# dwofk/fast-depth

Measured on NVIDIA H100. Metric: depth-maps/sec @224x224 b64, higher is better.
Workload: dtype f16

## Files before the change

### fastdepth_b200/_lib.py

```python
import ctypes
import os

HERE = os.path.dirname(os.path.abspath(__file__))
LIB_PATH = os.environ.get('FD_B200_LIB') or os.path.join(HERE, 'libfastdepth_b200.so')

FD_F32, FD_F16, FD_BF16 = 0, 1, 2
FD_STAGE_STEM, FD_STAGE_DWPW, FD_STAGE_HEAD, FD_STAGE_CONV, FD_STAGE_DECONV, FD_STAGE_UPCONV = 0, 1, 2, 3, 4, 5
FD_ACT_RELU, FD_ACT_RELU6 = 0, 1


class StageDesc(ctypes.Structure):
    _fields_ = [(n, ctypes.c_int32) for n in
                ('kind', 'c_in', 'c_out', 'ksize', 'stride', 'act', 'upsample', 'skip_src', 'skip_mode')]


_c_int_p = ctypes.POINTER(ctypes.c_int)
_c_float_p = ctypes.POINTER(ctypes.c_float)
_c_double_p = ctypes.POINTER(ctypes.c_double)
_vp = ctypes.c_void_p

SIGNATURES = {
    'fd_abi_version': (ctypes.c_int, []),
    'fd_last_error': (ctypes.c_char_p, []),
    'fd_plan_create': (ctypes.c_int, [ctypes.POINTER(StageDesc), ctypes.c_int, ctypes.c_int, ctypes.c_int,
# ... 9 lines not shown
    'fd_stage_buffer': (ctypes.c_int, [_vp, ctypes.c_int, ctypes.c_int, ctypes.POINTER(_vp),
                                       _c_int_p, _c_int_p, _c_int_p, _c_int_p, _c_int_p]),
    'fd_plan_launches_per_forward': (ctypes.c_int, [_vp, _c_int_p]),
    'fd_plan_workspace_bytes': (ctypes.c_int, [_vp, ctypes.POINTER(ctypes.c_size_t)]),
    'fd_plan_step_count': (ctypes.c_int, [_vp, _c_int_p]),
    'fd_plan_step_info': (ctypes.c_int, [_vp, ctypes.c_int, _c_int_p, _c_double_p, _c_double_p,
                                         ctypes.c_char_p, ctypes.c_int]),
    'fd_plan_step_macs': (ctypes.c_int, [_vp, ctypes.c_int, _c_double_p, _c_double_p]),
    'fd_plan_time_steps': (ctypes.c_int, [_vp, _vp, _vp, _vp, ctypes.c_int, ctypes.c_int, ctypes.c_int, _c_float_p]),
    'fd_plan_trace_stage': (ctypes.c_int, [_vp, ctypes.c_int, _vp, _vp, ctypes.POINTER(ctypes.c_uint64), ctypes.c_int,
                                           _c_int_p, _c_int_p]),
    'fd_debug_block_plan': (ctypes.c_int, [ctypes.c_int] * 8 + [_c_int_p, ctypes.c_int]),
    'fd_debug_conv_plan': (ctypes.c_int, [ctypes.c_int] * 7 + [_c_int_p, ctypes.c_int]),
    'fd_debug_convt_plan': (ctypes.c_int, [ctypes.c_int] * 8 + [_c_int_p, ctypes.c_int]),
    'fd_debug_pw_tf32x3_plan': (ctypes.c_int, [ctypes.c_int] * 7 + [_c_int_p, ctypes.c_int]),
    'fd_debug_conv_tf32x3_plan': (ctypes.c_int, [ctypes.c_int] * 9 + [_c_int_p, ctypes.c_int]),
    'fd_metrics_accumulate': (ctypes.c_int, [_vp, _vp, ctypes.c_int, ctypes.c_int, ctypes.c_int, _vp,
                                             ctypes.c_int, _vp]),
    'fd_nyu_val_gather': (ctypes.c_int, [_vp, _vp, _vp, _vp] + [ctypes.c_int] * 6 + [_vp, _vp, ctypes.c_int, _vp]),
    'fd_plan_destroy': (None, [_vp]),
}

_lib = None


def load():
    global _lib
    if _lib is not None:
        return _lib
    if not os.path.exists(LIB_PATH):
# ... 19 lines not shown
```

### fastdepth_b200/csrc/fd_api.cu

```cuda
#include <algorithm>
#include <cstring>
#include <functional>
#include <string>
#include <vector>

#include "fd_block_plan.h"
#include "fd_conv_plan.h"
#include "fd_common.cuh"

namespace fd {

BlockPlanOut block_tc_debug_plan(int ksize, int stride, int h_out, int w_out, int n, int c_in, int c_out, int head);
ConvPlanOut conv_tc_debug_plan(int kind, int ksize, int h_out, int w_out, int n, int c_in, int c_out, int n_sms);
ConvPlanOut pw_tf32x3_debug_plan(int h_out, int w_out, int n, int c_in, int c_out, int upsample, int n_sms);
ConvPlanOut conv_tc_tf32x3_debug_plan(int kind, int ksize, int h_out, int w_out, int n, int c_in, int c_out, int upsample,
                                      int n_sms);

static thread_local std::string g_last_error;
void set_error(const std::string& msg) { g_last_error = msg; }
int fail(int code, const std::string& msg) {
    g_last_error = msg;
    return code;
}

int launch_stem(int dtype, const void* x, void* out, const float* w, const float* scale, const float* bias,
                const StageGeom& g, cudaStream_t st);
int launch_dw(int dtype, const BlockArgs& a, cudaStream_t st);
int launch_pw(int dtype, const BlockArgs& a, cudaStream_t st);
int launch_conv(int dtype, const void* in, const void* w, void* out, const float* scale, const float* bias, const StageGeom& g,
// ... 29 lines not shown
const char* stem_tc_name(StemTcPlan* sp);
struct ConvTcPlan;
bool conv_tc_supported(int dtype, const StageGeom& g, int kind);
int conv_tc_prepare(int dtype, int kind, const StageGeom& g, const void* in, const void* w, const float* scale_dev,
                    const float* bias_dev, void* out, const TcLaunchOpts& opts, ConvTcPlan** res);
int conv_tc_launch(ConvTcPlan* cp, cudaStream_t st);
void conv_tc_destroy(ConvTcPlan* cp);
const char* conv_tc_name(ConvTcPlan* cp);
bool pw_tf32x3_supported(const StageGeom& g);
bool conv_tc_tf32x3_supported(const StageGeom& g, int kind);
int conv_tc_tf32x3_prepare(int kind, const StageGeom& g, const void* in, const float* w_split, const float* scale_dev,
                           const float* bias_dev, void* out, const TcLaunchOpts& opts, ConvTcPlan** res);
int pw_tf32x3_prepare(const StageGeom& g, const void* mid, const float* w_split, const float* scale_dev, const float* bias_dev,
                      void* out, int out_pitch, int reduce, const TcLaunchOpts& opts, ConvTcPlan** res);
int tf32_split_weights(const float* w, size_t count, float* dst);
size_t block_tc_param_bytes(BlockTcPlan* bp);
size_t chain_tc_param_bytes(ChainTcPlan* cp);
size_t stem_tc_param_bytes(StemTcPlan* sp);
size_t conv_tc_param_bytes(ConvTcPlan* cp);

static size_t dtype_size(int dtype) { return dtype == FD_F32 ? 4 : 2; }
static bool is_phased(int kind) { return kind == FD_STAGE_DECONV || kind == FD_STAGE_UPCONV; }
static bool is_conv(int kind) { return kind == FD_STAGE_CONV || is_phased(kind); }

struct Stage {
    fd_stage_desc d{};
    StageGeom g{};
    int out_h = 0, out_w = 0;
    void* out = nullptr;
    void* out_alloc = nullptr;
// ... 39 lines not shown
};

}

using namespace fd;

struct fd_plan {
    int n = 0, h = 0, w = 0, dtype = 0, device = 0, n_sms = 132;
    std::vector<Stage> stages;
    std::vector<StepSet*> sets;
    unsigned long long set_clock = 0;
    int opt_path = 1, opt_fold_head = 1, opt_graph = 1, opt_tma_epilogue = 1, opt_inplace_skip = 1, opt_pdl = 0, opt_wait_sleep_ns = 0;
    int opt_chain = 1;
    int opt_cluster = 1;
    int opt_tf32x3 = 0;
    size_t workspace_bytes = 0;
    size_t split_bytes = 0;
    struct PipeSlot { void* x = nullptr; void* y = nullptr; cudaEvent_t up = nullptr, done = nullptr, down = nullptr; bool busy = false; };
    PipeSlot pipe[3];
    cudaStream_t pipe_h2d = nullptr, pipe_run = nullptr, pipe_d2h = nullptr;
    unsigned long long pipe_next = 0;
    void* stage_x = nullptr;
    void* stage_y = nullptr;
    cudaEvent_t last_done = nullptr;
    cudaStream_t last_stream = nullptr;
    bool last_stream_set = false;
    void* l2_flush = nullptr;
    size_t l2_flush_bytes = 0;
    struct GraphEntry { const void* x; void* y; int n; cudaGraphExec_t exec; unsigned long long stamp; };
    std::vector<GraphEntry> graphs;
    unsigned long long graph_clock = 0;
    int graph_misses = 0;
};
static const size_t kMaxGraphs = 8;
static const size_t kMaxStepSets = 8;

namespace fd {

struct DeviceGuard {
    int prev = -1;
    bool ok = true;
    explicit DeviceGuard(int dev) {
        if (cudaGetDevice(&prev) != cudaSuccess) { ok = false; return; }
        if (prev != dev && cudaSetDevice(dev) != cudaSuccess) ok = false;
    }
    ~DeviceGuard() {
        if (prev >= 0) cudaSetDevice(prev);
    }
};
// ... 218 lines not shown
            a.in = in;
            a.mid = s.mid;
            a.out = s.out;
            a.skip = (s.d.skip_src >= 0 && !s.d.skip_mode) ? R[s.d.skip_src].out_eff : nullptr;
            a.dw_w = s.dw_w; a.dw_scale = s.dw_scale; a.dw_bias = s.dw_bias;
            a.pw_w = s.pw_w; a.pw_scale = s.pw_scale; a.pw_bias = s.pw_bias;
            const double px_in = (double)sg.n * sg.h_in * sg.w_in, px_out = (double)sg.n * sg.h_out * sg.w_out;
            const double up = a.g.upsample ? 4.0 : 1.0;
            const double dw_macs = px_out * sg.c_in * sg.ksize * sg.ksize, pw_macs = px_out * sg.c_in * sg.c_out;
            const double w_bytes = (double)sg.c_in * sg.ksize * sg.ksize * 4 + 2.0 * sg.c_in * 4 +
                                   (double)sg.c_in * sg.c_out * es + 2.0 * sg.c_out * 4;
            const double fused_bytes = (px_in * sg.c_in + px_out * up * sg.c_out * (a.skip ? 2.0 : 1.0)) * es + w_bytes;
            const int dtype = p->dtype;
            const bool fuse_head = folded_here && p->opt_path == 1 && block_tc_supported(dtype, a.g, true);
            bool use_tc = p->opt_path == 1 && block_tc_supported(dtype, a.g, false);
            if (use_tc) {
                const bool tma_epi = p->opt_tma_epilogue != 0;
                if (tma_epi && p->opt_inplace_skip && a.skip != nullptr) { a.out = const_cast<void*>(a.skip); r.out_eff = a.out; }
                int rc = fuse_head ? block_tc_prepare(dtype, a, head.pw_w_f32, head.head_scale, head.head_bias, head.g.act, nullptr, false, lopts, &r.tc)
                                   : block_tc_prepare(dtype, a, nullptr, 0.f, 0.f, 0, nullptr, tma_epi && (a.skip == nullptr || a.skip == a.out), lopts, &r.tc);
                if (rc != FD_OK) return rc;
                ss->bytes += block_tc_param_bytes(r.tc);
                Step st;
                st.stage = i;
                st.name = block_tc_name(r.tc);
                st.macs = dw_macs + pw_macs + (fuse_head ? px_out * sg.c_out : 0.0);
                st.dw_macs = dw_macs;
                st.alg_bytes = fuse_head ? (px_in * sg.c_in + px_out * 4.0) * es + w_bytes + sg.c_out * 4.0 : fused_bytes;
                BlockTcPlan* tc = r.tc;
                st.run = [tc](cudaStream_t stream, const void*, void* y) { return block_tc_launch(tc, stream, y); };
// ... 260 lines not shown
    return FD_OK;
}

static int* option_slot(fd_plan* p, const char* name) {
    if (!p || !name) return nullptr;
    if (!strcmp(name, "path")) return &p->opt_path;
    if (!strcmp(name, "fold_head")) return &p->opt_fold_head;
    if (!strcmp(name, "graph")) return &p->opt_graph;
    if (!strcmp(name, "tma_epilogue")) return &p->opt_tma_epilogue;
    if (!strcmp(name, "inplace_skip")) return &p->opt_inplace_skip;
    if (!strcmp(name, "pdl")) return &p->opt_pdl;
    if (!strcmp(name, "wait_sleep_ns")) return &p->opt_wait_sleep_ns;
    if (!strcmp(name, "chain")) return &p->opt_chain;
    if (!strcmp(name, "cluster")) return &p->opt_cluster;
    if (!strcmp(name, "tf32x3")) return &p->opt_tf32x3;
    return nullptr;
}

int fd_plan_set_option(fd_plan* p, const char* name, int value) {
    int* slot = option_slot(p, name);
    if (!slot) return fail(FD_ERR_INVALID, std::string("unknown option: ") + (name ? name : "(null)"));
    const bool is_time = !strcmp(name, "wait_sleep_ns");
    if (is_time ? (value < 0 || value > 100000) : (value != 0 && value != 1))
        return fail(FD_ERR_INVALID, is_time ? "wait_sleep_ns must be in [0, 100000]" : "option value must be 0 or 1");
    if (*slot != value) { *slot = value; invalidate(p); }
    return FD_OK;
}

int fd_plan_get_option(fd_plan* p, const char* name, int* value) {
    int* slot = option_slot(p, name);
    if (!slot || !value) return fail(FD_ERR_INVALID, "unknown option or NULL value");
    *value = *slot;
    return FD_OK;
}

static int ensure_steps(fd_plan* p, int n, StepSet** out) {
    StepSet* ss = find_set(p, n);
    if (!ss) {
        if (p->sets.size() >= kMaxStepSets) {
// ... 296 lines not shown
    const int v[16] = {q.ok, q.splits, q.n_cta, q.items, q.kblocks, q.s_in, q.s_a, q.s_b, q.bn, q.nb, q.b_resident, q.n_stg,
                       q.smem_bytes, q.in_stage_stride, q.cs, q.dw_teams};
    for (int i = 0; i < 16; ++i) out[i] = v[i];
    return FD_OK;
}

int fd_debug_conv_plan(int ksize, int h_out, int w_out, int n, int c_in, int c_out, int n_sms, int* out, int cap) {
    if (!out || cap < 16) return fail(FD_ERR_INVALID, "need an int[16] output");
    const ConvPlanOut q = conv_tc_debug_plan(FD_STAGE_CONV, ksize, h_out, w_out, n, c_in, c_out, n_sms);
    const int v[16] = {q.ok, q.ni, q.th, q.tw, q.bn, q.stages, q.m_tiles, q.n_splits, q.items, q.waves, q.kblocks, q.smem_bytes,
                       q.useful_permille, (int)(q.cost > 2e9 ? 2e9 : q.cost), 0, 0};
    for (int i = 0; i < 16; ++i) out[i] = v[i];
    return FD_OK;
}

int fd_debug_pw_tf32x3_plan(int h_out, int w_out, int n, int c_in, int c_out, int upsample, int n_sms, int* out, int cap) {
    if (!out || cap < 16) return fail(FD_ERR_INVALID, "need an int[16] output");
    const ConvPlanOut q = pw_tf32x3_debug_plan(h_out, w_out, n, c_in, c_out, upsample, n_sms);
    const int v[16] = {q.ok, q.ni, q.th, q.tw, q.bn, q.stages, q.m_tiles, q.n_splits, q.items, q.waves, q.kblocks, q.smem_bytes,
                       q.useful_permille, (int)(q.cost > 2e9 ? 2e9 : q.cost), q.ok ? conv_stage_bytes_tf32x3(q.bn) : 0, 0};
    for (int i = 0; i < 16; ++i) out[i] = v[i];
    return FD_OK;
}

int fd_debug_conv_tf32x3_plan(int kind, int ksize, int h, int w, int n, int c_in, int c_out, int upsample, int n_sms, int* out,
                              int cap) {
    if (!out || cap < 44) return fail(FD_ERR_INVALID, "need an int[44] output");
    if (kind != FD_STAGE_CONV && !is_phased(kind)) return fail(FD_ERR_INVALID, "kind must be FD_STAGE_CONV, FD_STAGE_DECONV or FD_STAGE_UPCONV");
    const ConvPlanOut q = conv_tc_tf32x3_debug_plan(kind, ksize, h, w, n, c_in, c_out, upsample, n_sms);
    const int v[16] = {q.ok, q.ni, q.th, q.tw, q.bn, q.stages, q.m_tiles, q.n_splits, q.items, q.waves, q.kblocks, q.smem_bytes,
// ... 70 lines not shown
```

### fastdepth_b200/csrc/fd_block_tc.cu

```cuda
#include <cuda.h>

#include <cstdio>
#include <cstdlib>
#include <cstring>
#include <new>
#include <string>

#include "fd_block_plan.h"
#include "fd_tc_common.cuh"

namespace fd {

constexpr int TC_DW_WARPS = 8;
constexpr int TC_EPI_WARPS = 8;
constexpr int TC_WARP_EPI0 = 0, TC_WARP_DW0 = TC_EPI_WARPS;
constexpr int TC_WARP_TMA = TC_DW_WARPS + TC_EPI_WARPS;
constexpr int TC_THREADS = (TC_WARP_TMA + 1) * 32;
constexpr int TC_WARP_BCAST = TC_WARP_TMA + 1;
constexpr int TC_THREADS_CL = (TC_WARP_BCAST + 1) * 32;
constexpr int TC_NCH = 2;
constexpr int TC_KBLK = 64;
constexpr int TC_A_STAGE_BYTES = 128 * 128;
constexpr int TC_MAX_IN = 6, TC_MAX_A = 6, TC_MAX_B = 16;
static_assert(TC_MAX_A >= kPlanMaxACluster && TC_MAX_A >= kPlanMaxA && TC_MAX_IN >= kPlanMaxIn && TC_MAX_B >= kPlanMaxB, "barrier arrays cover the planner's ring depths");
// ... 769 lines not shown
    if (i < n_dst) dst[i] = i < n_src ? src[i] : 0.f;
}

static int padded_copy(const float* src, int n_src, int n_dst, float** out) {
    FD_CUDA_OK(cudaMalloc(out, (size_t)n_dst * 4));
    pad_copy_kernel<<<(n_dst + 255) / 256, 256>>>(src, *out, n_src, n_dst);
    FD_CUDA_OK(cudaGetLastError());
    return FD_OK;
}

static int block_wmc_auto(const StageGeom& g, const BlockPlanOut& po, int n_tiles) {
    (void)g; (void)po; (void)n_tiles;
    return 1;
}

int block_tc_prepare(int dtype, const BlockArgs& a, const float* head_w, float head_scale, float head_bias, int head_act,
                     void* head_out, bool tma_epilogue, const TcLaunchOpts& opts, BlockTcPlan** out) {
    PFN_encodeTiled encode = get_encode();
    if (!encode) return fail(FD_ERR_CUDA, "cuTensorMapEncodeTiled is not available from this driver");
    const StageGeom& g = a.g;
    BlockTcPlan* bp = new (std::nothrow) BlockTcPlan();
    if (!bp) return fail(FD_ERR_CUDA, "out of host memory");
    bp->dtype = dtype; bp->ks = g.ksize; bp->stride = g.stride; bp->tile = pick_tile(g);
    bp->opts = opts;
    {
        const char* e = getenv("FD_TC_NO_HALFK");
        bp->halfk = (g.c_in <= 32 && g.ksize == 3 && g.stride == 1 && bp->tile == 0 && !(e && *e == '1')) ? 1 : 0;
    }
    const int NI = bp->tile ? 2 : 1, TH = 8, TW = bp->tile ? 8 : 16;
    const int IH = (TH - 1) * g.stride + g.ksize, IW = (TW - 1) * g.stride + g.ksize;
    TcParams& p = bp->p;
    memset(&p, 0, sizeof(p));
    p.n = g.n; p.h_in = g.h_in; p.w_in = g.w_in; p.h_out = g.h_out; p.w_out = g.w_out; p.c_in = g.c_in; p.c_out = g.c_out;
    p.tiles_x = (g.w_out + TW - 1) / TW; p.tiles_y = (g.h_out + TH - 1) / TH;
    const int tiles_img = (g.n + NI - 1) / NI;
    const int n_tiles = p.tiles_x * p.tiles_y * tiles_img;
    p.kblocks = (g.c_in + TC_KBLK - 1) / TC_KBLK; p.cin_pad = p.kblocks * TC_KBLK;
    p.act = g.act; p.upsample = g.upsample;
    p.head = head_w != nullptr; p.head_act = head_act; p.head_scale = head_scale; p.head_bias = head_bias;
    p.skip = a.skip; p.out = a.out; p.head_out = head_out;
    p.out_pitch = g.out_pitch > 0 ? g.out_pitch : g.c_out; p.skip_pitch = g.skip_pitch > 0 ? g.skip_pitch : g.c_out;
    const int in_pitch = g.in_pitch > 0 ? g.in_pitch : g.c_in;

    BlockPlanIn pin{};
    pin.ksize = g.ksize; pin.stride = g.stride; pin.tile = bp->tile; pin.c_in = g.c_in; pin.c_out = g.c_out; pin.n_tiles = n_tiles;
    pin.head = p.head; pin.barrier_bytes = (int)sizeof(TcBarriers); pin.n_sms = opts.n_sms;
    pin.cluster = (opts.cluster && !bp->halfk) ? 0 : 1;
    { const char* e = getenv("FD_TC_DW_TEAMS"); pin.even_rings = (e && *e == '1') ? 0 : ((e && *e == '2') ? 1 : 2); }
    if (pin.even_rings == 2 && g.ksize == 5 && (g.c_in + TC_KBLK - 1) / TC_KBLK <= 2) pin.even_rings = 1;
    plan_env_knobs(pin);
    if (bp->halfk) pin.cluster = 1;
    const BlockPlanOut po = plan_block(pin);
    if (!po.ok) { delete bp; return fail(FD_ERR_UNSUPPORTED, "fused block does not fit shared memory"); }
    const int splits = po.splits;
    p.n_cta = po.n_cta; p.splits = po.splits; p.items = po.items;
    p.in_stage_bytes = po.in_stage_bytes; p.dwp_bytes = po.dwp_bytes; p.in_stage_stride = po.in_stage_stride; p.cpad_all = po.cpad_all;
    p.s_a = po.s_a; p.n_stg = po.n_stg; p.s_in = po.s_in; p.s_b = po.s_b; p.bn = po.bn; p.nb = po.nb;
    p.b_resident = po.b_resident; p.b_stage_bytes = po.b_stage_bytes;
    p.cs = po.cs; bp->tiles = n_tiles;
    { const char* e = getenv("FD_TC_EPI_HIGH"); p.epi_high = (e && *e) ? atoi(e) : 0; }
    p.dw_teams = po.dw_teams;
    p.wmc = 1;
    {
        const char* e = getenv("FD_TC_WMC");
        int want = e && *e ? atoi(e) : 0;
        if (!opts.cluster || bp->halfk) want = 1;
        if (want == 0) want = block_wmc_auto(g, po, n_tiles);
// ... 96 lines not shown
```

### fastdepth_b200/csrc/fd_conv_plan.h

```cpp
#pragma once

namespace fd {

constexpr int kConvMaxStages = 8;
constexpr int kConvStg = 16384;
constexpr int kConvSmemBudget = 227 * 1024 - 128;
constexpr int kConvAlignSlack = 1024;
constexpr int kConvBarrierBytes = 256;

constexpr int kConvKindConv = 3, kConvKindDeconv = 4, kConvKindUpconv = 5;

struct ConvPhase { int tap0, ny, nx, dy0, dx0; };

inline int convt_tap(int kind, int k, int r, int d) {
    const int p = (k - 1) / 2;
    return kind == kConvKindDeconv ? r + p - 2 * d : 2 * d + p - r;
}

inline void convt_axis(int kind, int k, int r, int* d0, int* n) {
    const int p = (k - 1) / 2;
    int lo = 1 << 20, hi = -(1 << 20);
    for (int t = 0; t < k; ++t) {
        if ((t - r - p) & 1) continue;
        const int d = kind == kConvKindDeconv ? (r + p - t) / 2 : (r + t - p) / 2;
// ... 25 lines not shown
    int tf32x3;
};
struct ConvPlanOut {
    int ok;
    int ni, th, tw, bn, stages;
    int m_tiles, n_splits, items, waves, kblocks;
    int smem_bytes, useful_permille;
    double cost;
    int n_phases, groups;
    ConvPhase ph[4];
    int group_ph[4][2];
};

constexpr int kConvTiles[][3] = {{1, 8, 16}, {2, 8, 8}, {4, 4, 8}, {8, 4, 4}, {32, 2, 2}};
constexpr int kConvNumTiles = 5;

inline int conv_stage_bytes(int bn) { return 128 * 128 + bn * 128; }
inline int conv_stage_bytes_tf32x3(int bn) { return 128 * 128 + 2 * bn * 128; }
constexpr int kConvTf32x3MaxBn = 128;

inline ConvPlanOut plan_conv_one(const ConvPlanIn& q, int tile, int bn, int per_item) {
    ConvPlanOut o{};
    const int kind = q.kind ? q.kind : kConvKindConv;
    o.n_phases = conv_phases(kind, q.ksize, o.ph);
    for (int g = 0; g < 4; ++g) o.group_ph[g][0] = o.group_ph[g][1] = -1;
    if (o.n_phases == 1) {
        o.groups = 1; o.group_ph[0][0] = 0;
    } else if (per_item == 2) {
        const int t03 = o.ph[0].ny * o.ph[0].nx + o.ph[3].ny * o.ph[3].nx, t12 = o.ph[1].ny * o.ph[1].nx + o.ph[2].ny * o.ph[2].nx;
        o.groups = 2;
// ... 88 lines not shown
```

### fastdepth_b200/csrc/fd_conv_tc.cu

```cuda
#include <cstdint>
#include <cstdio>
#include <cstring>
#include <new>
#include <string>

#include "fd_conv_plan.h"
#include "fd_tc_common.cuh"

namespace fd {

constexpr int CV_WARP_TMA = 8, CV_THREADS = 288;
constexpr int CV_A_BYTES = 128 * 128;

struct ConvParams {
    int n, h, w, c_in, c_out;
    int ni, th, tw;
    int tiles_x, tiles_y, img_tiles, splits, items;
    int kblocks;
    int stages, stage_bytes;
    int upsample;
    int phased;
    ConvPhase ph[4];
    int group_code[4];
    unsigned long long mg_splits, mg_tx, mg_ty, mg_img;
// ... 13 lines not shown
    const uint32_t t2 = fdiv40(t, p.mg_tx);
    const int tx = (int)(t - t2 * (uint32_t)p.tiles_x);
    const uint32_t t3 = fdiv40(t2, p.mg_ty);
    const int ty = (int)(t2 - t3 * (uint32_t)p.tiles_y);
    const uint32_t t4 = fdiv40(t3, p.mg_img);
    c.code = p.group_code[t4];
    c.img0 = (int)(t3 - t4 * (uint32_t)p.img_tiles) * p.ni; c.oy0 = ty * p.th; c.ox0 = tx * p.tw; c.n0 = split * bn;
    return c;
}

template <typename T, int BN, bool RELU6>
__global__ void __launch_bounds__(CV_THREADS, 1)
conv_tc_kernel(const __grid_constant__ CUtensorMap tm_in, const __grid_constant__ CUtensorMap tm_w,
               const __grid_constant__ CUtensorMap tm_o0, const __grid_constant__ CUtensorMap tm_o1,
               const __grid_constant__ CUtensorMap tm_o2, const __grid_constant__ CUtensorMap tm_o3,
               const __grid_constant__ ConvParams p) {
    using MF = MixFma<T>;
    extern __shared__ uint8_t smem_raw[];
    const uint32_t smem_base = (smem_u32(smem_raw) + 1023u) & ~1023u;
    uint8_t* smem = smem_raw + (smem_base - smem_u32(smem_raw));
    const uint32_t stg_off = (uint32_t)p.stages * (uint32_t)p.stage_bytes;
    const uint32_t bar_off = stg_off + 2u * (uint32_t)kConvStg;
    ConvBarriers* bars = reinterpret_cast<ConvBarriers*>(smem + bar_off);
    const int warp = threadIdx.x >> 5, lane = threadIdx.x & 31;

    if (threadIdx.x == 0) {
        for (int i = 0; i < kConvMaxStages; ++i) { mbar_init(smem_u32(&bars->full[i]), 1); mbar_init(smem_u32(&bars->empty[i]), 2); }
        fence_barrier_init();
    }
    if (warp == CV_WARP_TMA && lane == 0) {
        tma_prefetch_desc(&tm_in); tma_prefetch_desc(&tm_w); tma_prefetch_desc(&tm_o0);
// ... 68 lines not shown
                        const f32x2 sc = f32x2_make(af.x, af.y), bi = f32x2_make(af.z, af.w);
#pragma unroll
                        for (int h = 0; h < 2; ++h) {
                            const int rr = r0 + 8 * h;
                            const int j = cb * 8 + i;
                            *reinterpret_cast<uint32_t*>(stg + rr * 128 + ((i ^ (rr & 7)) << 4) + cq * 2) =
                                MF::template pack_act<RELU6>(ffma2_abc(f32x2_make(acc[4 * j + 2 * h], acc[4 * j + 2 * h + 1]), sc, bi));
                        }
                    }
                    fence_proxy_async();
                    if (elected) bulk_wait_read0();
                    asm volatile("bar.sync %0, %1;" ::"r"(bar_id), "r"(bar_n) : "memory");
                    if (elected) {
                        const uint32_t src = smem_u32(stg);
                        const int cc = c.n0 + cb * 64;
                        tma_store_4d(q == 0 ? &tm_o0 : q == 1 ? &tm_o1 : q == 2 ? &tm_o2 : &tm_o3, src, cc, c.ox0, c.oy0, c.img0);
                        if (p.upsample) {
                            tma_store_4d(&tm_o1, src, cc, c.ox0, c.oy0, c.img0);
                            tma_store_4d(&tm_o2, src, cc, c.ox0, c.oy0, c.img0);
                            tma_store_4d(&tm_o3, src, cc, c.ox0, c.oy0, c.img0);
                        }
                        bulk_commit_group();
                    }
                }
            }
        }
        if (elected) bulk_wait_all();
    }
}

template <int BN, bool RELU6>
__global__ void __launch_bounds__(CV_THREADS, 1)
conv_tc_tf32x3_kernel(const __grid_constant__ CUtensorMap tm_in, const __grid_constant__ CUtensorMap tm_w,
                      const __grid_constant__ CUtensorMap tm_o0, const __grid_constant__ CUtensorMap tm_o1,
                      const __grid_constant__ CUtensorMap tm_o2, const __grid_constant__ CUtensorMap tm_o3,
// ... 113 lines not shown
                        const int v0 = p.phased ? q : 0, v1 = p.phased ? q + 1 : (p.upsample ? 4 : 1);
                        for (int v = v0; v < v1; ++v) {
                            const CUtensorMap* m = v == 0 ? &tm_o0 : v == 1 ? &tm_o1 : v == 2 ? &tm_o2 : &tm_o3;
                            if (reduce) tma_reduce_add_4d(m, src, cc, c.ox0, c.oy0, c.img0);
                            else tma_store_4d(m, src, cc, c.ox0, c.oy0, c.img0);
                        }
                        bulk_commit_group();
                    }
                }
            }
        }
        if (elected) bulk_wait_all();
    }
}

struct ConvTcPlan {
    CUtensorMap tm_in, tm_w, tm_o[4];
    ConvParams p;
    ConvPlanOut po;
    dim3 grid;
    size_t smem_bytes;
    int dtype, act;
    TcLaunchOpts opts;
    float2* affine = nullptr;
    size_t affine_bytes = 0;
    int tf32x3 = 0, reduce = 0;
    std::string name;
};

__global__ void split_tf32_kernel(const float* __restrict__ w, float* __restrict__ dst, int count) {
// ... 24 lines not shown
}

void conv_tc_destroy(ConvTcPlan* cp) {
    if (!cp) return;
    cudaFree(cp->affine);
    delete cp;
}

ConvPlanOut conv_tc_debug_plan(int kind, int ksize, int h_out, int w_out, int n, int c_in, int c_out, int n_sms) {
    ConvPlanIn q{};
    q.ksize = ksize; q.h_out = h_out; q.w_out = w_out; q.n = n; q.c_in = c_in; q.c_out = c_out; q.n_sms = n_sms;
    q.force_tile = -1; q.kind = kind;
    return plan_conv(q);
}

int conv_tc_prepare(int dtype, int kind, const StageGeom& g, const void* in, const void* w, const float* scale_dev,
                    const float* bias_dev, void* out, const TcLaunchOpts& opts, ConvTcPlan** res) {
    PFN_encodeTiled encode = get_tensor_map_encoder();
    if (!encode) return fail(FD_ERR_CUDA, "cuTensorMapEncodeTiled is not available from this driver");
    const bool phased = kind != kConvKindConv;
    ConvPlanIn q{};
    q.ksize = g.ksize; q.h_out = g.h_out; q.w_out = g.w_out; q.n = g.n; q.c_in = g.c_in; q.c_out = g.c_out; q.upsample = g.upsample;
    q.n_sms = opts.n_sms; q.force_tile = -1; q.kind = kind;
    { const char* e = getenv("FD_CONV_TILE"); if (e && *e) q.force_tile = atoi(e); }
    { const char* e = getenv("FD_CONV_BN"); if (e && *e) q.force_bn = atoi(e); }
    { const char* e = getenv("FD_CONV_PHASE_GROUP"); if (phased && e && *e) q.force_group = atoi(e); }
    const ConvPlanOut po = plan_conv(q);
    if (!po.ok) return fail(FD_ERR_UNSUPPORTED, "dense conv stage: no tile plan fits shared memory");
    ConvTcPlan* cp = new (std::nothrow) ConvTcPlan();
    if (!cp) return fail(FD_ERR_CUDA, "out of host memory");
    cp->dtype = dtype; cp->act = g.act; cp->opts = opts; cp->po = po;
    ConvParams& p = cp->p;
    memset(&p, 0, sizeof(p));
    p.n = g.n; p.h = g.h_out; p.w = g.w_out; p.c_in = g.c_in; p.c_out = g.c_out;
    p.ni = po.ni; p.th = po.th; p.tw = po.tw;
    p.tiles_x = (g.w_out + po.tw - 1) / po.tw; p.tiles_y = (g.h_out + po.th - 1) / po.th; p.img_tiles = (g.n + po.ni - 1) / po.ni;
    p.splits = po.n_splits; p.items = po.items;
    p.kblocks = po.kblocks;
    p.stages = po.stages; p.stage_bytes = conv_stage_bytes(po.bn);
    p.upsample = g.upsample; p.phased = phased ? 1 : 0;
    memcpy(p.ph, po.ph, sizeof(p.ph));
    for (int g = 0; g < 4; ++g) {
        p.group_code[g] = 0xF;
        for (int j = 1; j >= 0; --j)
            if (po.group_ph[g][j] >= 0) p.group_code[g] = (p.group_code[g] << 4) | po.group_ph[g][j];
    }
// ... 37 lines not shown
        for (int d = 0; d < (views4 ? 4 : 1); ++d) {
            char* base = reinterpret_cast<char*>(out) + ((size_t)(d >> 1) * W2 + (d & 1)) * P * es;
            cuuint64_t dims[4] = {(cuuint64_t)g.c_out, (cuuint64_t)g.w_out, (cuuint64_t)g.h_out, (cuuint64_t)g.n};
            cuuint64_t strides[3] = {up * P * es, up * W2 * P * es, H2 * W2 * P * es};
            cuuint32_t box[4] = {64, (cuuint32_t)po.tw, (cuuint32_t)po.th, (cuuint32_t)po.ni};
            cuuint32_t estr[4] = {1, 1, 1, 1};
            CUresult r = encode(&cp->tm_o[d], dt, 4, base, dims, strides, box, estr, CU_TENSOR_MAP_INTERLEAVE_NONE,
                                CU_TENSOR_MAP_SWIZZLE_128B, CU_TENSOR_MAP_L2_PROMOTION_L2_128B, CU_TENSOR_MAP_FLOAT_OOB_FILL_NONE);
            if (r != CUDA_SUCCESS) { conv_tc_destroy(cp); return fail(FD_ERR_CUDA, "cuTensorMapEncodeTiled(conv output) failed: " + std::to_string((int)r)); }
        }
    }
    cp->smem_bytes = (size_t)po.smem_bytes;
    cp->grid = dim3((unsigned)(p.items < opts.n_sms ? p.items : opts.n_sms), 1, 1);
    char buf[160];
    if (!phased)
        snprintf(buf, sizeof(buf), "conv_tc_kernel<k%d,bn%d,%s>[%dx%dx%d,n%d,st%d,%s]", g.ksize, po.bn, g.upsample ? "up" : "noup",
                 po.ni, po.th, po.tw, p.splits, p.stages, g.act == FD_ACT_RELU6 ? "relu6" : "relu");
    else
        snprintf(buf, sizeof(buf), "conv_tc_kernel<%s%d,bn%d,%s>[%dx%dx%d,n%d,st%d,%s]", kind == kConvKindDeconv ? "deconv" : "upconv",
                 g.ksize, po.bn, po.groups == 2 ? "4ph2" : "4ph", po.ni, po.th, po.tw, p.splits, p.stages,
                 g.act == FD_ACT_RELU6 ? "relu6" : "relu");
    cp->name = buf;
    *res = cp;
    return FD_OK;
}

bool pw_tf32x3_supported(const StageGeom& g) {
    return g.c_in % 8 == 0 && g.c_out % 8 == 0 && get_tensor_map_encoder() != nullptr;
}

bool conv_tc_tf32x3_supported(const StageGeom& g, int kind) {
    if (g.c_in % 8 || g.c_out % 8) return false;
    if (kind == kConvKindConv && ((g.ksize != 3 && g.ksize != 5) || g.stride != 1)) return false;
    if (kind == kConvKindDeconv && g.ksize != 3 && g.ksize != 5 && g.ksize != 7 && g.ksize != 9) return false;
    if (kind == kConvKindUpconv && g.ksize != 5) return false;
    return get_tensor_map_encoder() != nullptr;
}

ConvPlanOut pw_tf32x3_debug_plan(int h_out, int w_out, int n, int c_in, int c_out, int upsample, int n_sms) {
// ... 138 lines not shown
static int conv_launch_inst(ConvTcPlan* cp, cudaStream_t st) {
    auto kern = conv_tc_kernel<T, BN, RELU6>;
    static PerDeviceOnce attr_set;
    int dev = -1;
    FD_CUDA_OK(cudaGetDevice(&dev));
    if (attr_set.need(dev)) {
        FD_CUDA_OK(cudaFuncSetAttribute(kern, cudaFuncAttributeMaxDynamicSharedMemorySize, 227 * 1024));
        attr_set.done(dev);
    }
    cudaLaunchConfig_t cfg{};
    cfg.gridDim = cp->grid; cfg.blockDim = dim3(CV_THREADS); cfg.dynamicSmemBytes = cp->smem_bytes; cfg.stream = st;
    cudaLaunchAttribute attr[1];
    attr[0].id = cudaLaunchAttributeProgrammaticStreamSerialization;
    attr[0].val.programmaticStreamSerializationAllowed = 1;
    cfg.attrs = attr; cfg.numAttrs = cp->opts.pdl ? 1 : 0;
    FD_CUDA_OK(cudaLaunchKernelEx(&cfg, kern, cp->tm_in, cp->tm_w, cp->tm_o[0], cp->tm_o[1], cp->tm_o[2], cp->tm_o[3], cp->p));
    FD_CUDA_OK(cudaGetLastError());
    return FD_OK;
}

template <typename T>
static int conv_launch_t(ConvTcPlan* cp, cudaStream_t st) {
    const bool r6 = cp->act == FD_ACT_RELU6;
    switch (cp->po.bn) {
        case 64: return r6 ? conv_launch_inst<T, 64, true>(cp, st) : conv_launch_inst<T, 64, false>(cp, st);
        case 128: return r6 ? conv_launch_inst<T, 128, true>(cp, st) : conv_launch_inst<T, 128, false>(cp, st);
        case 256: return r6 ? conv_launch_inst<T, 256, true>(cp, st) : conv_launch_inst<T, 256, false>(cp, st);
        default: return fail(FD_ERR_UNSUPPORTED, "no conv_tc_kernel instance for this bn");
    }
}

// ... 38 lines not shown
```

### include/fastdepth_b200.h

```cpp
#ifndef FASTDEPTH_B200_H
#define FASTDEPTH_B200_H

#include <stddef.h>
#include <stdint.h>

#ifdef __cplusplus
extern "C" {
#endif

#define FD_ABI_VERSION 2

typedef struct fd_plan fd_plan;

typedef enum {
    FD_OK = 0,
    FD_ERR_INVALID = -1,
    FD_ERR_CUDA = -2,
    FD_ERR_STATE = -3,
    FD_ERR_UNSUPPORTED = -4
} fd_status;

typedef enum { FD_F32 = 0, FD_F16 = 1, FD_BF16 = 2 } fd_dtype;

typedef enum {
// ... 48 lines not shown
                      char* kernel_name, int name_cap);
int fd_plan_step_macs(fd_plan* plan, int step, double* dw_macs, double* dense_macs);
int fd_plan_time_steps(fd_plan* plan, const void* x_dev, void* y_dev, void* stream,
                       int warmup, int iters, int flush_l2, float* ms_out);

int fd_plan_trace_stage(fd_plan* plan, int stage, void* y_dev, void* stream,
                        unsigned long long* out_host, int cap, int* rows, int* cols);

int fd_debug_block_plan(int ksize, int stride, int h_out, int w_out, int n, int c_in, int c_out, int head,
                        int* out, int cap);

int fd_debug_conv_plan(int ksize, int h_out, int w_out, int n, int c_in, int c_out, int n_sms, int* out, int cap);

int fd_debug_pw_tf32x3_plan(int h_out, int w_out, int n, int c_in, int c_out, int upsample, int n_sms, int* out, int cap);

int fd_debug_convt_plan(int kind, int ksize, int h_in, int w_in, int n, int c_in, int c_out, int n_sms, int* out, int cap);

int fd_debug_conv_tf32x3_plan(int kind, int ksize, int h, int w, int n, int c_in, int c_out, int upsample, int n_sms,
                              int* out, int cap);

int fd_metrics_accumulate(const void* pred_dev, const float* target_dev, int dtype, int n, int hw,
                          double* sums_dev, int device, void* stream);

int fd_nyu_val_gather(const uint8_t* rgb_dev, const float* depth_dev, const int* rows_dev, const int* cols_dev,
                      int n, int h_in, int w_in, int out_h, int out_w, int dtype,
                      void* x_dev, float* target_dev, int device, void* stream);

void fd_plan_destroy(fd_plan* plan);

const char* fd_last_error(void);
// ... 7 lines not shown
```

Measured before the change: 53670.

## Unfuse wide depthwise-pointwise blocks into a depthwise kernel plus a flattened tensor-core GEMM

For depthwise-separable blocks whose fused plan would need many K-splits or cluster splitting, the block is now split into two kernels. A standalone CUDA-core depthwise kernel writes the intermediate activation to global memory. A flattened 1x1 tensor-core conv then reads it as a GEMM, with an optional TMA reduce-add epilogue that folds the skip connection in place. This is meant to avoid the fused kernel's inefficient split-K and tiling on wide layers. In exchange it adds a global round trip for the mid tensor, capped at 16 MB, plus an extra launch. The new path is enabled by default (unfuse=1).

```diff
diff --git a/fastdepth_b200/_lib.py b/fastdepth_b200/_lib.py
--- a/fastdepth_b200/_lib.py
+++ b/fastdepth_b200/_lib.py
@@ -47,6 +47,7 @@
     'fd_debug_conv_plan': (ctypes.c_int, [ctypes.c_int] * 7 + [_c_int_p, ctypes.c_int]),
     'fd_debug_convt_plan': (ctypes.c_int, [ctypes.c_int] * 8 + [_c_int_p, ctypes.c_int]),
     'fd_debug_pw_tf32x3_plan': (ctypes.c_int, [ctypes.c_int] * 7 + [_c_int_p, ctypes.c_int]),
+    'fd_debug_pw_plan': (ctypes.c_int, [ctypes.c_int] * 7 + [_c_int_p, ctypes.c_int]),
     'fd_debug_conv_tf32x3_plan': (ctypes.c_int, [ctypes.c_int] * 9 + [_c_int_p, ctypes.c_int]),
     'fd_metrics_accumulate': (ctypes.c_int, [_vp, _vp, ctypes.c_int, ctypes.c_int, ctypes.c_int, _vp,
                                              ctypes.c_int, _vp]),
diff --git a/fastdepth_b200/csrc/fd_api.cu b/fastdepth_b200/csrc/fd_api.cu
--- a/fastdepth_b200/csrc/fd_api.cu
+++ b/fastdepth_b200/csrc/fd_api.cu
@@ -13,6 +13,7 @@
 BlockPlanOut block_tc_debug_plan(int ksize, int stride, int h_out, int w_out, int n, int c_in, int c_out, int head);
 ConvPlanOut conv_tc_debug_plan(int kind, int ksize, int h_out, int w_out, int n, int c_in, int c_out, int n_sms);
 ConvPlanOut pw_tf32x3_debug_plan(int h_out, int w_out, int n, int c_in, int c_out, int upsample, int n_sms);
+ConvPlanOut pw_tc_debug_plan(int h_out, int w_out, int n, int c_in, int c_out, int upsample, int n_sms);
 ConvPlanOut conv_tc_tf32x3_debug_plan(int kind, int ksize, int h_out, int w_out, int n, int c_in, int c_out, int upsample,
                                       int n_sms);
 
@@ -72,6 +73,11 @@
 int pw_tf32x3_prepare(const StageGeom& g, const void* mid, const float* w_split, const float* scale_dev, const float* bias_dev,
                       void* out, int out_pitch, int reduce, const TcLaunchOpts& opts, ConvTcPlan** res);
 int tf32_split_weights(const float* w, size_t count, float* dst);
+bool pw_tc_supported(int dtype, const StageGeom& g);
+int pw_tc_prepare(int dtype, const StageGeom& g, const void* mid, const void* w, const float* scale_dev, const float* bias_dev,
+                  void* out, int out_pitch, int reduce, const TcLaunchOpts& opts, ConvTcPlan** res);
+int dw_mid_launch(int dtype, const BlockArgs& a, cudaStream_t st);
+BlockPlanOut block_tc_plan_for(const StageGeom& g, const TcLaunchOpts& opts, bool* pinned);
 size_t block_tc_param_bytes(BlockTcPlan* bp);
 size_t chain_tc_param_bytes(ChainTcPlan* cp);
 size_t stem_tc_param_bytes(StemTcPlan* sp);
@@ -141,6 +147,7 @@
     int opt_chain = 1;
     int opt_cluster = 1;
     int opt_tf32x3 = 0;
+    int opt_unfuse = 1;
     size_t workspace_bytes = 0;
     size_t split_bytes = 0;
     struct PipeSlot { void* x = nullptr; void* y = nullptr; cudaEvent_t up = nullptr, done = nullptr, down = nullptr; bool busy = false; };
@@ -160,6 +167,7 @@
     int graph_misses = 0;
 };
 static const size_t kMaxGraphs = 8;
+static const size_t kUnfuseMaxMidBytes = size_t(16) << 20;
 static const size_t kMaxStepSets = 8;
 
 namespace fd {
@@ -408,6 +416,39 @@
             const int dtype = p->dtype;
             const bool fuse_head = folded_here && p->opt_path == 1 && block_tc_supported(dtype, a.g, true);
             bool use_tc = p->opt_path == 1 && block_tc_supported(dtype, a.g, false);
+            const bool add_in_place = a.skip != nullptr && p->opt_tma_epilogue && p->opt_inplace_skip;
+            if (use_tc && p->opt_unfuse && !folded_here && (a.skip == nullptr || add_in_place) && pw_tc_supported(dtype, a.g)) {
+                bool pinned = false;
+                const BlockPlanOut bpo = block_tc_plan_for(a.g, lopts, &pinned);
+                const size_t mid_bytes = (size_t)px_out * sg.c_in * dtype_size(dtype);
+                const bool wide = bpo.ok && (bpo.splits >= 8 || bpo.cs > 1) && mid_bytes <= kUnfuseMaxMidBytes;
+                if (!pinned && (p->opt_unfuse == 2 || wide)) {
+                    void* out = a.skip ? const_cast<void*>(a.skip) : a.out;
+                    const int opitch = a.skip ? a.g.skip_pitch : a.g.out_pitch;
+                    if (a.skip) r.out_eff = out;
+                    int rc = pw_tc_prepare(dtype, a.g, a.mid, a.pw_w, a.pw_scale, a.pw_bias, out, opitch, a.skip ? 1 : 0, lopts, &r.ctc);
+                    if (rc != FD_OK) return rc;
+                    ss->bytes += conv_tc_param_bytes(r.ctc);
+                    Step d;
+                    d.stage = i;
+                    d.name = sg.ksize == 3 ? "dw_mid_kernel<3>" : "dw_mid_kernel<5>";
+                    d.macs = dw_macs;
+                    d.dw_macs = dw_macs;
+                    d.alg_bytes = (px_in + px_out) * sg.c_in * es + (double)sg.c_in * (sg.ksize * sg.ksize + 2) * 4;
+                    d.run = [a, dtype](cudaStream_t stream, const void*, void*) { return dw_mid_launch(dtype, a, stream); };
+                    ss->steps.push_back(d);
+                    Step q;
+                    q.stage = i;
+                    q.name = std::string("pw:") + conv_tc_name(r.ctc);
+                    q.macs = pw_macs;
+                    q.alg_bytes = (px_out * sg.c_in + px_out * up * sg.c_out * (a.skip ? 2.0 : 1.0)) * es +
+                                  (double)sg.c_in * sg.c_out * es + 2.0 * sg.c_out * 4;
+                    ConvTcPlan* ctc = r.ctc;
+                    q.run = [ctc](cudaStream_t stream, const void*, void*) { return conv_tc_launch(ctc, stream); };
+                    ss->steps.push_back(q);
+                    continue;
+                }
+            }
             if (use_tc) {
                 const bool tma_epi = p->opt_tma_epilogue != 0;
                 if (tma_epi && p->opt_inplace_skip && a.skip != nullptr) { a.out = const_cast<void*>(a.skip); r.out_eff = a.out; }
@@ -698,6 +739,7 @@
     if (!strcmp(name, "chain")) return &p->opt_chain;
     if (!strcmp(name, "cluster")) return &p->opt_cluster;
     if (!strcmp(name, "tf32x3")) return &p->opt_tf32x3;
+    if (!strcmp(name, "unfuse")) return &p->opt_unfuse;
     return nullptr;
 }
 
@@ -705,8 +747,11 @@
     int* slot = option_slot(p, name);
     if (!slot) return fail(FD_ERR_INVALID, std::string("unknown option: ") + (name ? name : "(null)"));
     const bool is_time = !strcmp(name, "wait_sleep_ns");
-    if (is_time ? (value < 0 || value > 100000) : (value != 0 && value != 1))
+    if (!strcmp(name, "unfuse")) {
+        if (value < 0 || value > 2) return fail(FD_ERR_INVALID, "unfuse must be 0, 1 or 2");
+    } else if (is_time ? (value < 0 || value > 100000) : (value != 0 && value != 1)) {
         return fail(FD_ERR_INVALID, is_time ? "wait_sleep_ns must be in [0, 100000]" : "option value must be 0 or 1");
+    }
     if (*slot != value) { *slot = value; invalidate(p); }
     return FD_OK;
 }
@@ -1033,6 +1078,15 @@
     return FD_OK;
 }
 
+int fd_debug_pw_plan(int h_out, int w_out, int n, int c_in, int c_out, int upsample, int n_sms, int* out, int cap) {
+    if (!out || cap < 16) return fail(FD_ERR_INVALID, "need an int[16] output");
+    const ConvPlanOut q = pw_tc_debug_plan(h_out, w_out, n, c_in, c_out, upsample, n_sms);
+    const int v[16] = {q.ok, q.ni, q.th, q.tw, q.bn, q.stages, q.m_tiles, q.n_splits, q.items, q.waves, q.kblocks, q.smem_bytes,
+                       q.useful_permille, (int)(q.cost > 2e9 ? 2e9 : q.cost), q.ok ? conv_stage_bytes(q.bn) : 0, 0};
+    for (int i = 0; i < 16; ++i) out[i] = v[i];
+    return FD_OK;
+}
+
 int fd_debug_pw_tf32x3_plan(int h_out, int w_out, int n, int c_in, int c_out, int upsample, int n_sms, int* out, int cap) {
     if (!out || cap < 16) return fail(FD_ERR_INVALID, "need an int[16] output");
     const ConvPlanOut q = pw_tf32x3_debug_plan(h_out, w_out, n, c_in, c_out, upsample, n_sms);
diff --git a/fastdepth_b200/csrc/fd_block_tc.cu b/fastdepth_b200/csrc/fd_block_tc.cu
--- a/fastdepth_b200/csrc/fd_block_tc.cu
+++ b/fastdepth_b200/csrc/fd_block_tc.cu
@@ -807,6 +807,30 @@
     return 1;
 }
 
+static BlockPlanIn block_plan_in(const StageGeom& g, int tile, int halfk, int n_tiles, int head, const TcLaunchOpts& opts) {
+    BlockPlanIn pin{};
+    pin.ksize = g.ksize; pin.stride = g.stride; pin.tile = tile; pin.c_in = g.c_in; pin.c_out = g.c_out; pin.n_tiles = n_tiles;
+    pin.head = head; pin.barrier_bytes = (int)sizeof(TcBarriers); pin.n_sms = opts.n_sms;
+    pin.cluster = (opts.cluster && !halfk) ? 0 : 1;
+    { const char* e = getenv("FD_TC_DW_TEAMS"); pin.even_rings = (e && *e == '1') ? 0 : ((e && *e == '2') ? 1 : 2); }
+    if (pin.even_rings == 2 && g.ksize == 5 && (g.c_in + TC_KBLK - 1) / TC_KBLK <= 2) pin.even_rings = 1;
+    plan_env_knobs(pin);
+    if (halfk) pin.cluster = 1;
+    return pin;
+}
+
+BlockPlanOut block_tc_plan_for(const StageGeom& g, const TcLaunchOpts& opts, bool* pinned) {
+    const int tile = pick_tile(g);
+    const int NI = tile ? 2 : 1, TW = tile ? 8 : 16;
+    const int n_tiles = ((g.w_out + TW - 1) / TW) * ((g.h_out + 7) / 8) * ((g.n + NI - 1) / NI);
+    const char* e = getenv("FD_TC_NO_HALFK");
+    const int halfk = (g.c_in <= 32 && g.ksize == 3 && g.stride == 1 && tile == 0 && !(e && *e == '1')) ? 1 : 0;
+    const BlockPlanIn pin = block_plan_in(g, tile, halfk, n_tiles, 0, opts);
+    auto set = [](const char* name) { const char* v = getenv(name); return v && *v; };
+    *pinned = pin.max_n_cta > 0 || pin.cluster >= 2 || set("FD_TC_WMC") || set("FD_TC_DW_TEAMS");
+    return plan_block(pin);
+}
+
 int block_tc_prepare(int dtype, const BlockArgs& a, const float* head_w, float head_scale, float head_bias, int head_act,
                      void* head_out, bool tma_epilogue, const TcLaunchOpts& opts, BlockTcPlan** out) {
     PFN_encodeTiled encode = get_encode();
@@ -835,15 +859,7 @@
     p.out_pitch = g.out_pitch > 0 ? g.out_pitch : g.c_out; p.skip_pitch = g.skip_pitch > 0 ? g.skip_pitch : g.c_out;
     const int in_pitch = g.in_pitch > 0 ? g.in_pitch : g.c_in;
 
-    BlockPlanIn pin{};
-    pin.ksize = g.ksize; pin.stride = g.stride; pin.tile = bp->tile; pin.c_in = g.c_in; pin.c_out = g.c_out; pin.n_tiles = n_tiles;
-    pin.head = p.head; pin.barrier_bytes = (int)sizeof(TcBarriers); pin.n_sms = opts.n_sms;
-    pin.cluster = (opts.cluster && !bp->halfk) ? 0 : 1;
-    { const char* e = getenv("FD_TC_DW_TEAMS"); pin.even_rings = (e && *e == '1') ? 0 : ((e && *e == '2') ? 1 : 2); }
-    if (pin.even_rings == 2 && g.ksize == 5 && (g.c_in + TC_KBLK - 1) / TC_KBLK <= 2) pin.even_rings = 1;
-    plan_env_knobs(pin);
-    if (bp->halfk) pin.cluster = 1;
-    const BlockPlanOut po = plan_block(pin);
+    const BlockPlanOut po = plan_block(block_plan_in(g, bp->tile, bp->halfk, n_tiles, p.head, opts));
     if (!po.ok) { delete bp; return fail(FD_ERR_UNSUPPORTED, "fused block does not fit shared memory"); }
     const int splits = po.splits;
     p.n_cta = po.n_cta; p.splits = po.splits; p.items = po.items;
diff --git a/fastdepth_b200/csrc/fd_conv_plan.h b/fastdepth_b200/csrc/fd_conv_plan.h
--- a/fastdepth_b200/csrc/fd_conv_plan.h
+++ b/fastdepth_b200/csrc/fd_conv_plan.h
@@ -63,6 +63,13 @@
 
 constexpr int kConvTiles[][3] = {{1, 8, 16}, {2, 8, 8}, {4, 4, 8}, {8, 4, 4}, {32, 2, 2}};
 constexpr int kConvNumTiles = 5;
+
+inline bool conv_flat_rows(int upsample, int* n, int* h, int* w) {
+    const long long m = (long long)*n * *h * *w;
+    if (upsample || m % 16 || m / 128 >= (1 << 18)) return false;
+    *n = 1; *h = (int)(m / 16); *w = 16;
+    return true;
+}
 
 inline int conv_stage_bytes(int bn) { return 128 * 128 + bn * 128; }
 inline int conv_stage_bytes_tf32x3(int bn) { return 128 * 128 + 2 * bn * 128; }
diff --git a/fastdepth_b200/csrc/fd_conv_tc.cu b/fastdepth_b200/csrc/fd_conv_tc.cu
--- a/fastdepth_b200/csrc/fd_conv_tc.cu
+++ b/fastdepth_b200/csrc/fd_conv_tc.cu
@@ -3,6 +3,7 @@
 #include <cstring>
 #include <new>
 #include <string>
+#include <type_traits>
 
 #include "fd_conv_plan.h"
 #include "fd_tc_common.cuh"
@@ -51,7 +52,7 @@
 conv_tc_kernel(const __grid_constant__ CUtensorMap tm_in, const __grid_constant__ CUtensorMap tm_w,
                const __grid_constant__ CUtensorMap tm_o0, const __grid_constant__ CUtensorMap tm_o1,
                const __grid_constant__ CUtensorMap tm_o2, const __grid_constant__ CUtensorMap tm_o3,
-               const __grid_constant__ ConvParams p) {
+               const __grid_constant__ ConvParams p, const int reduce) {
     using MF = MixFma<T>;
     extern __shared__ uint8_t smem_raw[];
     const uint32_t smem_base = (smem_u32(smem_raw) + 1023u) & ~1023u;
@@ -150,11 +151,20 @@
                     if (elected) {
                         const uint32_t src = smem_u32(stg);
                         const int cc = c.n0 + cb * 64;
-                        tma_store_4d(q == 0 ? &tm_o0 : q == 1 ? &tm_o1 : q == 2 ? &tm_o2 : &tm_o3, src, cc, c.ox0, c.oy0, c.img0);
-                        if (p.upsample) {
-                            tma_store_4d(&tm_o1, src, cc, c.ox0, c.oy0, c.img0);
-                            tma_store_4d(&tm_o2, src, cc, c.ox0, c.oy0, c.img0);
-                            tma_store_4d(&tm_o3, src, cc, c.ox0, c.oy0, c.img0);
+                        if (reduce) {
+                            tma_reduce_add_4d(&tm_o0, src, cc, c.ox0, c.oy0, c.img0);
+                            if (p.upsample) {
+                                tma_reduce_add_4d(&tm_o1, src, cc, c.ox0, c.oy0, c.img0);
+                                tma_reduce_add_4d(&tm_o2, src, cc, c.ox0, c.oy0, c.img0);
+                                tma_reduce_add_4d(&tm_o3, src, cc, c.ox0, c.oy0, c.img0);
+                            }
+                        } else {
+                            tma_store_4d(q == 0 ? &tm_o0 : q == 1 ? &tm_o1 : q == 2 ? &tm_o2 : &tm_o3, src, cc, c.ox0, c.oy0, c.img0);
+                            if (p.upsample) {
+                                tma_store_4d(&tm_o1, src, cc, c.ox0, c.oy0, c.img0);
+                                tma_store_4d(&tm_o2, src, cc, c.ox0, c.oy0, c.img0);
+                                tma_store_4d(&tm_o3, src, cc, c.ox0, c.oy0, c.img0);
+                            }
                         }
                         bulk_commit_group();
                     }
@@ -298,6 +308,76 @@
     }
 }
 
+template <typename T, int K, bool RELU6, int PX>
+__global__ void __launch_bounds__(256)
+dw_mid_kernel(const T* __restrict__ in, T* __restrict__ mid, const float* __restrict__ w, const float* __restrict__ scale,
+              const float* __restrict__ bias, int n, int h_in, int w_in, int h_out, int w_out, int c, int in_pitch, int stride) {
+    using MF = MixFma<T>;
+    const int groups = c >> 3, segs = (w_out + PX - 1) / PX;
+    const long long total = (long long)n * h_out * segs * groups;
+    const long long idx = (long long)blockIdx.x * blockDim.x + threadIdx.x;
+    if (idx >= total) return;
+    const int g = (int)(idx % groups);
+    long long t = idx / groups;
+    const int ox0 = (int)(t % segs) * PX;
+    const int oy = (int)((t / segs) % h_out);
+    const int img = (int)(t / ((long long)segs * h_out));
+    constexpr int PAD = (K - 1) / 2;
+    auto rt = [](float v) { return Traits<T>::to_f(Traits<T>::from_f(v)); };
+    f32x2 acc[PX][4];
+#pragma unroll
+    for (int o = 0; o < PX; ++o)
+#pragma unroll
+        for (int j = 0; j < 4; ++j) acc[o][j] = 0ull;
+    const T* base = in + (size_t)img * h_in * w_in * in_pitch + g * 8;
+    auto row = [&](auto stride_c, int ky) {
+        constexpr int S = decltype(stride_c)::value;
+        const int iy = oy * S - PAD + ky;
+        if (iy < 0 || iy >= h_in) return;
+        f32x2 wk[K][4];
+#pragma unroll
+        for (int kx = 0; kx < K; ++kx) {
+            const float4* wp = reinterpret_cast<const float4*>(w + (size_t)(ky * K + kx) * c + g * 8);
+            const float4 w0 = __ldg(wp), w1 = __ldg(wp + 1);
+            wk[kx][0] = f32x2_make(rt(w0.x), rt(w0.y)); wk[kx][1] = f32x2_make(rt(w0.z), rt(w0.w));
+            wk[kx][2] = f32x2_make(rt(w1.x), rt(w1.y)); wk[kx][3] = f32x2_make(rt(w1.z), rt(w1.w));
+        }
+#pragma unroll
+        for (int j = 0; j < (PX - 1) * S + K; ++j) {
+            const int ix = ox0 * S - PAD + j;
+            if (ix < 0 || ix >= w_in) continue;
+            const uint4 v = __ldg(reinterpret_cast<const uint4*>(base + ((size_t)iy * w_in + ix) * in_pitch));
+            const f32x2 x0 = MF::widen(v.x), x1 = MF::widen(v.y), x2 = MF::widen(v.z), x3 = MF::widen(v.w);
+#pragma unroll
+            for (int o = 0; o < PX; ++o) {
+                const int kx = j - o * S;
+                if (kx < 0 || kx >= K) continue;
+                ffma2(acc[o][0], x0, wk[kx][0]); ffma2(acc[o][1], x1, wk[kx][1]);
+                ffma2(acc[o][2], x2, wk[kx][2]); ffma2(acc[o][3], x3, wk[kx][3]);
+            }
+        }
+    };
+#pragma unroll
+    for (int ky = 0; ky < K; ++ky) {
+        if (stride == 1) row(std::integral_constant<int, 1>(), ky);
+        else row(std::integral_constant<int, 2>(), ky);
+    }
+    const float4* sp = reinterpret_cast<const float4*>(scale + g * 8);
+    const float4* bp = reinterpret_cast<const float4*>(bias + g * 8);
+    const float4 s0 = __ldg(sp), s1 = __ldg(sp + 1), b0 = __ldg(bp), b1 = __ldg(bp + 1);
+    T* orow = mid + (((size_t)img * h_out + oy) * w_out) * c + g * 8;
+#pragma unroll
+    for (int o = 0; o < PX; ++o) {
+        if (ox0 + o >= w_out) break;
+        uint4 r;
+        r.x = MF::template pack_act<RELU6>(ffma2_abc(acc[o][0], f32x2_make(s0.x, s0.y), f32x2_make(b0.x, b0.y)));
+        r.y = MF::template pack_act<RELU6>(ffma2_abc(acc[o][1], f32x2_make(s0.z, s0.w), f32x2_make(b0.z, b0.w)));
+        r.z = MF::template pack_act<RELU6>(ffma2_abc(acc[o][2], f32x2_make(s1.x, s1.y), f32x2_make(b1.x, b1.y)));
+        r.w = MF::template pack_act<RELU6>(ffma2_abc(acc[o][3], f32x2_make(s1.z, s1.w), f32x2_make(b1.z, b1.w)));
+        *reinterpret_cast<uint4*>(orow + (size_t)(ox0 + o) * c) = r;
+    }
+}
+
 struct ConvTcPlan {
     CUtensorMap tm_in, tm_w, tm_o[4];
     ConvParams p;
@@ -352,8 +432,8 @@
     return plan_conv(q);
 }
 
-int conv_tc_prepare(int dtype, int kind, const StageGeom& g, const void* in, const void* w, const float* scale_dev,
-                    const float* bias_dev, void* out, const TcLaunchOpts& opts, ConvTcPlan** res) {
+static int conv_prepare(int dtype, int kind, const StageGeom& g, const void* in, const void* w, const float* scale_dev,
+                        const float* bias_dev, void* out, int reduce, const TcLaunchOpts& opts, ConvTcPlan** res) {
     PFN_encodeTiled encode = get_tensor_map_encoder();
     if (!encode) return fail(FD_ERR_CUDA, "cuTensorMapEncodeTiled is not available from this driver");
     const bool phased = kind != kConvKindConv;
@@ -367,7 +447,7 @@
     if (!po.ok) return fail(FD_ERR_UNSUPPORTED, "dense conv stage: no tile plan fits shared memory");
     ConvTcPlan* cp = new (std::nothrow) ConvTcPlan();
     if (!cp) return fail(FD_ERR_CUDA, "out of host memory");
-    cp->dtype = dtype; cp->act = g.act; cp->opts = opts; cp->po = po;
+    cp->dtype = dtype; cp->act = g.act; cp->opts = opts; cp->po = po; cp->reduce = reduce;
     ConvParams& p = cp->p;
     memset(&p, 0, sizeof(p));
     p.n = g.n; p.h = g.h_out; p.w = g.w_out; p.c_in = g.c_in; p.c_out = g.c_out;
@@ -435,8 +515,8 @@
     cp->grid = dim3((unsigned)(p.items < opts.n_sms ? p.items : opts.n_sms), 1, 1);
     char buf[160];
     if (!phased)
-        snprintf(buf, sizeof(buf), "conv_tc_kernel<k%d,bn%d,%s>[%dx%dx%d,n%d,st%d,%s]", g.ksize, po.bn, g.upsample ? "up" : "noup",
-                 po.ni, po.th, po.tw, p.splits, p.stages, g.act == FD_ACT_RELU6 ? "relu6" : "relu");
+        snprintf(buf, sizeof(buf), "conv_tc_kernel<k%d,bn%d,%s>[%dx%dx%d,n%d,st%d,%s%s]", g.ksize, po.bn, g.upsample ? "up" : "noup",
+                 po.ni, po.th, po.tw, p.splits, p.stages, g.act == FD_ACT_RELU6 ? "relu6" : "relu", reduce ? ",+skip(red)" : "");
     else
         snprintf(buf, sizeof(buf), "conv_tc_kernel<%s%d,bn%d,%s>[%dx%dx%d,n%d,st%d,%s]", kind == kConvKindDeconv ? "deconv" : "upconv",
                  g.ksize, po.bn, po.groups == 2 ? "4ph2" : "4ph", po.ni, po.th, po.tw, p.splits, p.stages,
@@ -444,6 +524,60 @@
     cp->name = buf;
     *res = cp;
     return FD_OK;
+}
+
+int conv_tc_prepare(int dtype, int kind, const StageGeom& g, const void* in, const void* w, const float* scale_dev,
+                    const float* bias_dev, void* out, const TcLaunchOpts& opts, ConvTcPlan** res) {
+    return conv_prepare(dtype, kind, g, in, w, scale_dev, bias_dev, out, 0, opts, res);
+}
+
+bool pw_tc_supported(int dtype, const StageGeom& g) {
+    if (dtype != FD_F16 && dtype != FD_BF16) return false;
+    return g.c_in % 8 == 0 && g.c_out % 8 == 0 && get_tensor_map_encoder() != nullptr;
+}
+
+static StageGeom pw_geom(const StageGeom& g, int out_pitch) {
+    StageGeom q = g;
+    q.ksize = 1; q.stride = 1;
+    conv_flat_rows(q.upsample, &q.n, &q.h_out, &q.w_out);
+    q.h_in = q.h_out; q.w_in = q.w_out; q.in_pitch = g.c_in; q.out_pitch = out_pitch;
+    return q;
+}
+
+ConvPlanOut pw_tc_debug_plan(int h_out, int w_out, int n, int c_in, int c_out, int upsample, int n_sms) {
+    ConvPlanIn q{};
+    q.ksize = 1; q.h_out = h_out; q.w_out = w_out; q.n = n; q.c_in = c_in; q.c_out = c_out; q.upsample = upsample;
+    q.n_sms = n_sms; q.force_tile = -1; q.kind = kConvKindConv;
+    conv_flat_rows(upsample, &q.n, &q.h_out, &q.w_out);
+    return plan_conv(q);
+}
+
+int pw_tc_prepare(int dtype, const StageGeom& g, const void* mid, const void* w, const float* scale_dev, const float* bias_dev,
+                  void* out, int out_pitch, int reduce, const TcLaunchOpts& opts, ConvTcPlan** res) {
+    return conv_prepare(dtype, kConvKindConv, pw_geom(g, out_pitch), mid, w, scale_dev, bias_dev, out, reduce, opts, res);
+}
+
+template <typename T, int PX>
+static int dw_mid_launch_t(const BlockArgs& a, cudaStream_t st) {
+    const StageGeom& g = a.g;
+    const long long total = (long long)g.n * g.h_out * ((g.w_out + PX - 1) / PX) * (g.c_in / 8);
+    const unsigned blocks = (unsigned)((total + 255) / 256);
+    const int in_pitch = g.in_pitch > 0 ? g.in_pitch : g.c_in;
+    const bool r6 = g.act == FD_ACT_RELU6;
+#define FD_DW_MID(K, R6)                                                                                                           \
+    dw_mid_kernel<T, K, R6, PX><<<blocks, 256, 0, st>>>(static_cast<const T*>(a.in), static_cast<T*>(a.mid), a.dw_w, a.dw_scale,  \
+                                                        a.dw_bias, g.n, g.h_in, g.w_in, g.h_out, g.w_out, g.c_in, in_pitch, g.stride)
+    if (g.ksize == 3) { if (r6) FD_DW_MID(3, true); else FD_DW_MID(3, false); }
+    else if (g.ksize == 5) { if (r6) FD_DW_MID(5, true); else FD_DW_MID(5, false); }
+    else return fail(FD_ERR_UNSUPPORTED, "no dw_mid_kernel instance for this kernel size");
+#undef FD_DW_MID
+    FD_CUDA_OK(cudaGetLastError());
+    return FD_OK;
+}
+
+int dw_mid_launch(int dtype, const BlockArgs& a, cudaStream_t st) {
+    if (dtype != FD_F16 && dtype != FD_BF16) return fail(FD_ERR_UNSUPPORTED, "dw_mid_kernel is a 16-bit kernel");
+    return dtype == FD_F16 ? dw_mid_launch_t<__half, 4>(a, st) : dw_mid_launch_t<__nv_bfloat16, 4>(a, st);
 }
 
 bool pw_tf32x3_supported(const StageGeom& g) {
@@ -612,7 +746,8 @@
     attr[0].id = cudaLaunchAttributeProgrammaticStreamSerialization;
     attr[0].val.programmaticStreamSerializationAllowed = 1;
     cfg.attrs = attr; cfg.numAttrs = cp->opts.pdl ? 1 : 0;
-    FD_CUDA_OK(cudaLaunchKernelEx(&cfg, kern, cp->tm_in, cp->tm_w, cp->tm_o[0], cp->tm_o[1], cp->tm_o[2], cp->tm_o[3], cp->p));
+    FD_CUDA_OK(cudaLaunchKernelEx(&cfg, kern, cp->tm_in, cp->tm_w, cp->tm_o[0], cp->tm_o[1], cp->tm_o[2], cp->tm_o[3], cp->p,
+                                  cp->reduce));
     FD_CUDA_OK(cudaGetLastError());
     return FD_OK;
 }
diff --git a/include/fastdepth_b200.h b/include/fastdepth_b200.h
--- a/include/fastdepth_b200.h
+++ b/include/fastdepth_b200.h
@@ -86,6 +86,8 @@
 
 int fd_debug_pw_tf32x3_plan(int h_out, int w_out, int n, int c_in, int c_out, int upsample, int n_sms, int* out, int cap);
 
+int fd_debug_pw_plan(int h_out, int w_out, int n, int c_in, int c_out, int upsample, int n_sms, int* out, int cap);
+
 int fd_debug_convt_plan(int kind, int ksize, int h_in, int w_in, int n, int c_in, int c_out, int n_sms, int* out, int cap);
 
 int fd_debug_conv_tf32x3_plan(int kind, int ksize, int h, int w, int n, int c_in, int c_out, int upsample, int n_sms,
```

Result: faster. 55680 (median of 6 runs) (+3.7%).
